# yoshihikosuzuki/ClassPro

Hardware: AMD Instinct MI355X
Metric: Mbases/s classified (k=40, 40x HiFi) at 1/2/4/8 MI355X vs CPU -T16 (higher is better)
Workload: dtype u16/f64

## Files before the change

### classpro_amd/csrc/capi.hip

```cpp
#include <hip/hip_runtime.h>
#include <stdio.h>
#include <stdlib.h>
#include <string.h>
#include <string>
#include <mutex>
#include <vector>
#include <chrono>
#include <thread>
#include <type_traits>
#include <time.h>
#include "cp_host_setup.h"
#include "kernels.hip"

static thread_local std::string g_err;
static int set_err(int code, const std::string &msg) { g_err = msg; return code; }

#define HIPCHK(call)                                                                       \
  do { hipError_t e_ = (call);                                                             \
       if (e_ != hipSuccess)                                                               \
         return set_err(CP_EHIP,std::string(#call)+": "+hipGetErrorString(e_));            \
     } while (0)
static int launch_status() { HIPCHK(hipGetLastError()); return CP_OK; }

extern "C" const char *cp_last_error(void) { return g_err.c_str(); }
// ... 966 lines not shown
  return CP_OK;
}
#endif

#if defined(CP_SEED_DEBUG) || defined(CP_SEED_DEBUG_TAKES)
extern "C" int cp_debug_seed_set(int read)
{ HIPCHK(hipMemcpyToSymbol(HIP_SYMBOL(g_seed_dbg_read),&read,sizeof(int))); return CP_OK; }
extern "C" int cp_debug_seed_get(int *out4, int *recs)
{ HIPCHK(hipDeviceSynchronize());
  HIPCHK(hipMemcpyFromSymbol(out4,HIP_SYMBOL(g_seed_dbg_n),16));
  HIPCHK(hipMemcpyFromSymbol(recs,HIP_SYMBOL(g_seed_dbg),8192*16));
  return CP_OK;
}
#endif
#if defined(CP_SEED_PROF) || defined(CP_PROF_WALK)
static int prof_read(unsigned long long *out, const void *sym, size_t n, bool reset = true)
{ static const unsigned long long z[13] = {0};
  HIPCHK(hipMemcpyFromSymbol(out,sym,n*sizeof(unsigned long long)));
  if (reset) HIPCHK(hipMemcpyToSymbol(sym,z,n*sizeof(unsigned long long)));
  return CP_OK;
}
#endif
#ifdef CP_SEED_PROF
extern "C" int cp_debug_seed_prof(unsigned long long *out8)
{ HIPCHK(hipDeviceSynchronize()); return prof_read(out8,HIP_SYMBOL(g_seed_prof),8); }
#endif
extern "C" int cp_debug_task_counts(cp_workspace *ws, int32_t *out, int64_t nreads)
{ if (!ws || !out || nreads < 0 || nreads > ws->nreads || ws->b.fwc.cap < (size_t)nreads*16)
    return set_err(CP_EINVAL,"cp_debug_task_counts: bad arguments");
  HIPCHK(hipDeviceSynchronize());
  if (nreads > 0) HIPCHK(hipMemcpy(out,ws->b.fwc.p,(size_t)nreads*4*sizeof(int32_t),hipMemcpyDeviceToHost));
  return CP_OK;
}
extern "C" int cp_debug_flag_bytes(cp_workspace *ws, int64_t *out2)
{ if (!ws || !out2) return set_err(CP_EINVAL,"cp_debug_flag_bytes: bad arguments");
  HIPCHK(hipDeviceSynchronize());
  const dbuf *arr[2] = { &ws->b.wall, &ws->b.wall_s };
  for (int a = 0; a < 2; a++)
    { std::vector<uint8_t> h(arr[a]->cap);
      if (arr[a]->cap) HIPCHK(hipMemcpy(h.data(),arr[a]->p,arr[a]->cap,hipMemcpyDeviceToHost));
      int64_t n = 0;
      for (uint8_t v : h) n += v != 0;
      out2[a] = n;
    }
  return CP_OK;
}
#ifdef CP_PROF_WALK
extern "C" int cp_debug_live_prof(unsigned long long *out8)
{ HIPCHK(hipDeviceSynchronize()); return prof_read(out8,HIP_SYMBOL(g_live_prof),8); }
extern "C" int cp_debug_emit_prof(unsigned long long *out8)
{ HIPCHK(hipDeviceSynchronize()); return prof_read(out8,HIP_SYMBOL(g_emit_prof),8); }
extern "C" int cp_debug_fw_prof(unsigned long long *out12)
{ HIPCHK(hipDeviceSynchronize()); return prof_read(out12,HIP_SYMBOL(g_fw_prof),12); }
extern "C" int cp_debug_unrel_prof(unsigned long long *out12)
{ HIPCHK(hipDeviceSynchronize()); return prof_read(out12,HIP_SYMBOL(g_unrel_prof),12); }
extern "C" int cp_debug_rel_prof(unsigned long long *out13)
{ HIPCHK(hipDeviceSynchronize()); return prof_read(out13,HIP_SYMBOL(g_rel_prof),13); }
extern "C" int cp_debug_phase_prof(unsigned long long *out36)
{ HIPCHK(hipDeviceSynchronize());
  CHK(prof_read(out36,HIP_SYMBOL(g_phase_max),12));
  CHK(prof_read(out36+12,HIP_SYMBOL(g_phase_sum),12));
  return prof_read(out36+24,HIP_SYMBOL(g_phase_arg),12,false);
}
#endif

#include "kmer_table.hip"

#include "kmer_counts.hip"

#include "kmer_sort.hip"

#include "kmer_lookup.hip"

#include "kmer_hits.hip"

#include "kmer_runs.hip"

#include "kmer_setops.hip"

#include "kmer_cmphist.hip"

#include "kmer_hetpairs.hip"

#include "kmer_unitigs.hip"

#include "kmer_unitig_graph.hip"

#include "kmer_paths.hip"

#include "kmer_prune.hip"

#include "label_tools.hip"
```

### classpro_amd/csrc/cp_wall.h

```cpp
#pragma once
#include "cp_math.h"
#include "cp_ctx.h"

#ifndef CP_HDM
#ifdef __HIPCC__
#define CP_HDM __host__ __device__ __forceinline__
#else
#define CP_HDM inline
#endif
#endif
#include "cp_bounds.h"

struct cp_perr_dense
  { double *a;
    CP_HDM double get(int pos, int e, int w) const { return a[(size_t)pos*4+e*2+w]; }
    CP_HDM void   set(int pos, int e, int w, double v) { a[(size_t)pos*4+e*2+w] = v; }
    CP_HDM long long cell(int pos, int e, int w) { return (long long)pos*4+e*2+w; }
    CP_HDM double    load(long long c) const { return a[c]; }
    CP_HDM void      store(long long c, double v) { a[c] = v; }
  };

struct cp_perr_hash
  { int32_t *keys;
    double  *vals;
// ... 96 lines not shown
    int                  eidx, oidx;
    int                  overflow;
    int                  use_win = 0, win_base = 0;
    uint64_t             win_lo = 0, win_hi = 0;
    int                  spec_wallnow = 0;
  };

#if defined(CP_PROF_WALK) && defined(__HIP_DEVICE_COMPILE__)
extern __device__ unsigned long long g_live_prof[8];
extern __device__ unsigned long long g_emit_prof[8];
#endif
#if defined(CP_PROF_WALK) && defined(CP_PROF_INNER) && defined(__HIP_DEVICE_COMPILE__)
#define CP_LT(k) do { unsigned long long t_ = wall_clock64(); if (__ffsll((long long)__ballot(1))-1 == (int)(threadIdx.x & 63)) atomicAdd(&g_live_prof[k],t_-lt_); lt_ = wall_clock64(); } while (0)
#define CP_LT0() unsigned long long lt_ = wall_clock64()
#define CP_ET(k) do { unsigned long long t_ = wall_clock64(); if (__ffsll((long long)__ballot(1))-1 == (int)(threadIdx.x & 63)) atomicAdd(&g_emit_prof[k],t_-et_); et_ = wall_clock64(); } while (0)
#define CP_ET0() unsigned long long et_ = wall_clock64()
#else
#define CP_LT(k) ((void)0)
#define CP_LT0() ((void)0)
#define CP_ET(k) ((void)0)
#define CP_ET0() ((void)0)
#endif

#define CP_PERR(R,i,e,w) ((R)->perror.get(i,e,w))
#define CP_NEG_INF (-INFINITY)

template <class RD>
CP_HD void cp_update_perror(RD *R, int i, int e, int w, int cout, int cin, double erate, double lpe, double l1mpe)
{ if (CP_PERR(R,i,e,w) == CP_NEG_INF)
    R->perror.set(i,e,w,cp_p_errorin(R->lf,e,erate,lpe,l1mpe,cout,cin));
}

template <class RD>
CP_HD double cp_logp_diff_pair(const RD *R, int i, int j)
{ const auto &pr = R->prof;
  int n_drop = (int)pr[i-1]-pr[i];
  int n_gain = (int)pr[j]-pr[j-1];
  int cov    = pr[i-1] > pr[j] ? pr[i-1] : pr[j];
  return cp_logp_trans(R->P,i,j,n_drop,n_gain,cov);
}

struct __attribute__((packed, aligned(2))) cp_u16x8 { uint16_t v[8]; };
template <class PROF>
CP_HD cp_u16x8 cp_load_u16x8(const PROF &prof, int lo) { return *reinterpret_cast<const cp_u16x8 *>(CP_SPAN(prof,lo,8)); }

struct __attribute__((packed, aligned(2))) cp_u16x8w { uint32_t w[4]; };
template <class PROF>
CP_HD cp_u16x8w cp_load_u16x8w(const PROF &prof, int lo) { return *reinterpret_cast<const cp_u16x8w *>(CP_SPAN(prof,lo,8)); }
CP_HD int cp_u16x8_get(const cp_u16x8w &x, int q) { return (int)((x.w[q >> 1] >> (16*(q & 1))) & 0xffffu); }

CP_HD bool cp_cthres_ng(int e, int cin, int ct)
{ return (e == CP_SELF) ? (cin >= ct) : (cin < ct); }

struct cp_wall_pre
  { int    cng, wtype, cin, cout, maxt, maxl;
    double maxpe, lpe, l1mpe;
  };

#define CP_CF_LIVE     1
#define CP_CF_WALLNOW  2
#define CP_LC_NONE     0
#define CP_LC_BOUNDARY 1
#define CP_LC_PAIR     2
#define CP_LC_REJECT   3

struct cp_cand_pure
  { double own_pe;
    double lc_v;
    double hc_pe;
    int    lc_j, hc_j;
    int    flags, lc_kind;
  };

template <class RD>
CP_HD void cp_wall_candidate_pre(const RD *R, int i, cp_wall_pre *pre)
{ const cp_dev_params *P = R->P;
  const int cim1 = R->prof[i-1], ci = R->prof[i];
  int cng = cim1-ci;
  if (cng < 0) cng = -cng;
  pre->cng = cng;
  if (cim1 > ci) { pre->wtype = CP_DROP; pre->cin = ci;   pre->cout = cim1; }
  else           { pre->wtype = CP_GAIN; pre->cin = cim1; pre->cout = ci;   }
  int maxt = -1, maxl = -1;
  double maxpe = CP_NEG_INF;
  int l3[3];
  cp_ctx3(R->seq,R->rlen,P->K,pre->wtype,i,l3);
  for (int t = 0; t < 3; t++)
    { int l = l3[t];
      if (l > P->lmax[t]) l = P->lmax[t];
      double pe = P->pe[t][l];
      if (maxpe < pe)
        { maxpe = pe; maxt = t; maxl = l; }
    }
  pre->maxt = maxt; pre->maxl = maxl; pre->maxpe = maxpe;
  pre->lpe = P->lpe[maxt][maxl];
  pre->l1mpe = P->l1mpe[maxt][maxl];
}

CP_HD int cp_wall_candidate_filter(const cp_dev_params *P, int e, const cp_wall_pre &pre)
{ const int CMAX = P->cmax;
  const int cng = pre.cng, cin = pre.cin, cout = pre.cout;
  int ct_init = 0, ct_final = 0;
  if (cout < CMAX)
    { ct_init  = P->cthres[pre.maxt][pre.maxl][cout][CP_INIT][e];
      ct_final = P->cthres[pre.maxt][pre.maxl][cout][CP_FINAL][e];
      if (!(cng > CP_MAX_CNT_CHANGE || cin < (ct_init > 3 ? ct_init : 3)))
        return 0;
    }
  if (e == CP_SELF)
    { if (cout < CMAX && cin >= ct_final)
        return 0;
    }
  else if (cng >= P->cov[CP_HAPLO] || (cout < CMAX && cin < ct_final))
    return CP_CF_WALLNOW;
  return CP_CF_LIVE;
}

struct cp_no_prep { CP_HDM void operator()() const {} };
template <class RD, class PREP>
CP_HD void cp_wall_candidate_live(RD *R, int i, int e, const cp_wall_pre &pre, cp_cand_pure *out, PREP prep)
{ const cp_dev_params *P = R->P;
  const auto &pr = R->prof;
  const int plen = R->plen, K = P->K, CMAX = P->cmax;
  const int w = pre.wtype, cin = pre.cin, cout = pre.cout;
  const int t = pre.maxt, l = pre.maxl;
  out->flags = CP_CF_LIVE; out->lc_kind = CP_LC_NONE; out->lc_j = -1; out->hc_j = -1;
  out->lc_v = out->hc_pe = CP_NEG_INF;
  CP_LT0();
  const int ulen = t+1;
  const bool right = (w == CP_DROP);
  int n, j, cout_j, cin_j;

  const double *nowhere = &P->pe[0][0];
  const double *petab = P->petab;
  const int pe_cmax = P->pe_cmax;
  const double *own_at = cp_p_errorin_at(petab,pe_cmax,e,t,l,cout,cin);
  const double *pei_at = cp_p_errorin_at(petab,pe_cmax,e,CP_HP,1,cout,cin);
  const double own_ld = cp_load_table(own_at ? own_at : nowhere), pei_ld = cp_load_table(pei_at ? pei_at : nowhere);
  const int    thr_i  = P->cthres[CP_HP][1][cout < CMAX ? cout : 0][CP_FINAL][e];
  cp_u16x8w cx;
  const int j0 = right ? (i+K-1) : (i-K+1);
  const int lo8 = right ? j0-2 : j0-(CP_MAX_N_HC+1);
  const bool wide = lo8 >= 0 && lo8+8 <= plen;
  cx.w[0] = cx.w[1] = cx.w[2] = cx.w[3] = 0;
  if (wide) cx = cp_load_u16x8w(pr,lo8);
  prep();
  CP_LT(0);

  const int m = ulen*l;
  n = 0;
  while (true)
    { int idx = right ? i+ulen*(n+1) : i-ulen*(n+1);
      if (right ? (idx >= plen) : (idx <= 0))
        break;
      if (cp_ctx(R->seq,R->rlen,K,w,idx,t) != m+n+1)
        break;
      n++;
    }
  CP_LT(1);
  out->own_pe = own_at ? own_ld : cp_p_errorin_calc(P,e,t,l,cout,cin);
  const int dlc = n-m;
  j = right ? j0+dlc : j0-dlc;
  if (right ? (j <= i) : (j >= i))
    return;

  constexpr int NP = CP_MAX_N_HC+2;
  int pj[NP], pcin[NP], pcout[NP], cw[8];
#ifdef __HIPCC__
// ... 586 lines not shown
```

### classpro_amd/csrc/kernels.hip

```cpp
#include <hip/hip_runtime.h>
#include <stdint.h>
#include <type_traits>
#include "cp_wall.h"
#include "cp_class.h"
#include "cp_seed.h"

#ifdef CP_BOUNDS
__device__ unsigned long long g_bounds[4];
#endif
#define WAVE 64
#define REL_MAXM 1024
#define UNREL_MAXN 1024
#ifndef REL_SMALL_MAXM
#define REL_SMALL_MAXM 112
#endif
#ifndef UNREL_SMALL_MAXN
#define UNREL_SMALL_MAXN 256
#endif
#define GRP_MAX_PLEN 65535

__device__ __forceinline__ void wave_sync() { __syncthreads(); }
__device__ __forceinline__ void wave_sync_lds()
{ __builtin_amdgcn_fence(__ATOMIC_RELEASE,"wavefront"); __builtin_amdgcn_wave_barrier(); __builtin_amdgcn_fence(__ATOMIC_ACQUIRE,"wavefront"); }

__device__ __forceinline__ int lane_id() { return threadIdx.x & (WAVE-1); }
__device__ __forceinline__ int wave_from_below(int v, int first) { return __builtin_amdgcn_update_dpp(first,v,0x138,0xf,0xf,false); }
__device__ __forceinline__ int wave_of_last(int v) { return __builtin_amdgcn_readlane(v,WAVE-1); }

typedef unsigned cp_u4v __attribute__((ext_vector_type(4)));
#ifndef SCAN_PLAIN
__device__ __forceinline__ uint4 scan_load(const uint4 *p)
{ cp_u4v x = __builtin_nontemporal_load(reinterpret_cast<const cp_u4v *>(p)); return make_uint4(x.x,x.y,x.z,x.w); }
#define SCAN_LOAD(p) scan_load(p)
#define SCAN_STORE(p,v) __builtin_nontemporal_store((uint8_t)(v),(p))
#else
#define SCAN_LOAD(p) (*(p))
#define SCAN_STORE(p,v) (*(p) = (uint8_t)(v))
#endif
#ifndef SCAN_UNROLL
#define SCAN_UNROLL 4
#endif
#ifndef SCAN_BLOCKS_PER_CU
#define SCAN_BLOCKS_PER_CU 8
#endif

typedef unsigned short cp_us2 __attribute__((ext_vector_type(2)));
__device__ __forceinline__ unsigned scan_pair_flags(unsigned prevcur, unsigned cur, int rep)
{ const cp_us2 a = __builtin_bit_cast(cp_us2,prevcur), b = __builtin_bit_cast(cp_us2,cur);
  const cp_us2 mn = __builtin_elementwise_min(a,b), mx = __builtin_elementwise_max(a,b);
  const cp_us2 r2 = { (unsigned short)rep, (unsigned short)rep }, two = { 2, 2 }, one = { 1, 1 };
  const cp_us2 s1 = __builtin_elementwise_sub_sat(r2,mn);
  const cp_us2 s2 = __builtin_elementwise_sub_sat((cp_us2)(mx-mn),two);
  const cp_us2 m = __builtin_elementwise_min(__builtin_elementwise_min(s1,s2),one);
  return __builtin_bit_cast(unsigned,m);
}

__global__ void __launch_bounds__(256)
k_scan_candidates(const uint16_t *__restrict__ prof, int64_t total, int rep, uint8_t *__restrict__ bitmap, int64_t nbytes, int has_prev)
{
  const int64_t ngroups = total >> 3;
  const int64_t nthreads = (int64_t)gridDim.x*blockDim.x;
  const int lane = lane_id();
  const uint4 *vp = reinterpret_cast<const uint4 *>(prof);

#ifndef SCAN_INTERLEAVED
  const int64_t wavesz = (int64_t)WAVE*SCAN_UNROLL;
  const int64_t nwaves = nthreads/WAVE;
  const int64_t wid = ((int64_t)blockIdx.x*blockDim.x+threadIdx.x)/WAVE;
  for (int64_t base = wid*wavesz; base < ngroups; base += nwaves*wavesz)
    { uint4 v[SCAN_UNROLL];
      int64_t g[SCAN_UNROLL];
#pragma unroll
      for (int u = 0; u < SCAN_UNROLL; u++)
        { g[u] = base+(int64_t)u*WAVE+lane;
          v[u] = (g[u] < ngroups) ? SCAN_LOAD(&vp[g[u]]) : make_uint4(0,0,0,0);
        }
      unsigned carry = 0;
      if (lane == 0)
        carry = (base > 0 || has_prev) ? prof[base*8-1] : (v[0].x & 0xffff);
#pragma unroll
// ... 17 lines not shown
      int64_t g[SCAN_UNROLL];
#pragma unroll
      for (int u = 0; u < SCAN_UNROLL; u++)
        { g[u] = base+(int64_t)u*blockDim.x+threadIdx.x;
          if (g[u] < ngroups)
            v[u] = SCAN_LOAD(&vp[g[u]]);
          else
            v[u] = make_uint4(0,0,0,0);
        }
#pragma unroll
      for (int u = 0; u < SCAN_UNROLL; u++)
        { const bool live = g[u] < ngroups;
          unsigned last = v[u].w >> 16;
          unsigned prev = __shfl_up(last,1);
          if (lane == 0 && live)
            prev = (g[u] > 0 || has_prev) ? prof[g[u]*8-1] : (v[u].x & 0xffff);
          unsigned c[8] = { v[u].x & 0xffff, v[u].x >> 16, v[u].y & 0xffff, v[u].y >> 16,
                            v[u].z & 0xffff, v[u].z >> 16, v[u].w & 0xffff, v[u].w >> 16 };
          unsigned bits = 0;
#pragma unroll
          for (int k = 0; k < 8; k++)
            { unsigned a = prev, b = c[k];
              unsigned mn = a < b ? a : b, df = a < b ? b-a : a-b;
              bits |= ((mn < (unsigned)rep) && (df >= CP_MIN_CNT_CHANGE)) ? (1u << k) : 0u;
              prev = b;
            }
          if (live)
            SCAN_STORE(&bitmap[g[u]],bits);
        }
    }

#endif

  if (blockIdx.x == 0 && threadIdx.x == 0)
    { int64_t p0 = ngroups << 3;
      if (p0 < total)
        { unsigned bits = 0;
          for (int64_t p = p0; p < total; p++)
            if (p > 0 || has_prev)
              { unsigned a = prof[p-1], b = prof[p];
                unsigned mn = a < b ? a : b, df = a < b ? b-a : a-b;
                if (mn < (unsigned)rep && df >= CP_MIN_CNT_CHANGE) bits |= 1u << (p-p0);
              }
          bitmap[ngroups] = (uint8_t)bits;
          p0 += 8;
        }
      for (int64_t q = p0 >> 3; q < nbytes; q++)
        bitmap[q] = 0;
    }
}

__device__ __forceinline__ uint64_t bitmap_word(const uint64_t *bm, int64_t w, int64_t lo, int64_t hi)
{
  uint64_t x = bm[w];
  int64_t w0 = w << 6;
  if (lo > w0)      x &= ~0ull << (lo-w0);
  if (hi < w0+64)   x &= (hi <= w0) ? 0ull : (~0ull >> (w0+64-hi));
  return x;
}

__global__ void __launch_bounds__(WAVE)
k_count_caps(const uint64_t *__restrict__ bm, const int64_t *__restrict__ prof_off, int nreads,
             int32_t *__restrict__ ncand, int64_t *__restrict__ icap, int64_t *__restrict__ ecap,
             int64_t *__restrict__ hcap)
{ const int r = blockIdx.x;
  if (r >= nreads) return;
  const int lane = lane_id();
  const int64_t lo = prof_off[r]+1, hi = prof_off[r+1];
  int cnt = 0;
  if (hi > lo)
    for (int64_t w = (lo >> 6)+lane; w <= ((hi-1) >> 6); w += WAVE)
      cnt += __popcll(bitmap_word(bm,w,lo,hi));
  for (int o = 32; o > 0; o >>= 1)
    cnt += __shfl_xor(cnt,o);
  if (lane == 0)
    { ncand[r] = cnt;
      icap[r]  = 2*(int64_t)cnt+4;
      ecap[r]  = 16*(int64_t)cnt+64;
      int64_t h = 32;
      while (h < 4*(int64_t)cnt+16) h <<= 1;
      hcap[r] = 2*h;
    }
}

template <class T>
__device__ __forceinline__ T block_scan_excl_256(T x, T *tmp, T *total)
{ const int t = threadIdx.x, lane = t & 63, wv = t >> 6;
  T inc = x;
  for (int o = 1; o < WAVE; o <<= 1)
    { T y = __shfl_up(inc,o); if (lane >= o) inc += y; }
  __syncthreads();
  if (lane == WAVE-1) tmp[wv] = inc;
  __syncthreads();
  T base = 0, all = 0;
#pragma unroll
  for (int w = 0; w < 4; w++) { const T v = tmp[w]; if (w < wv) base += v; all += v; }
  *total = all;
  return base+inc-x;
}

#define SCAN_TILE 1024
#define SCAN_TAG_BITS 24
#define SCAN_TAG_MASK 0xffffffull
struct cp_scan_state { unsigned long long g[3]; unsigned long long pad_; };
__global__ void __launch_bounds__(WAVE)
k_prefix_caps_mb(int64_t *__restrict__ a, int64_t *__restrict__ b, int64_t *__restrict__ c, int n, int64_t *__restrict__ totals,
                 cp_scan_state *__restrict__ state, int epoch, unsigned long long *__restrict__ host_tot)
{ const int t = threadIdx.x, tile = blockIdx.x, i0 = tile*SCAN_TILE+16*t;
  int64_t *arr[3] = { a, b, c };
  int64_t off[3], sum[3], pre[3];
#pragma unroll
// ... 447 lines not shown
          if (mv != ~0ull) break;
        }
      if (nx > 0 && !done && !flush_x(right ? 0x7fffffff : -1)) return;
      if (!done && (right ? plen < jend : jend == 0))
        { const double pe = pe_i * pe_i;
          if (pe >= CP_PE_THRES_FINAL)
            { if (*midx >= R->ecap) { R->overflow = 1; return; }
              ev.wave_grow(*midx);
              if (lane == 0)
                { cp_eintvl x; x.b = right ? i : 0; x.e = right ? plen : i; x.pe = pe;
                  ev.put(*midx,x);
                  F.fo[q] |= CP_W_PAIRED_M;
                }
              (*midx)++;
              if (*midx >= plen) { R->overflow = 8; return; }
            }
        }
      wave_sync();
    }
}

#define CP_PCLS(e,a)   (((uint32_t)(e) << 3) | ((uint32_t)(a) & 7u))
#define CP_PCLS_END(x) ((int)((x) >> 3))
#define CP_PCLS_CLS(x) (((x) & 7u) == 7u ? -1 : (int)((x) & 7u))

struct cp_rrec { int32_t b, e; uint16_t ccb, cce; int32_t idx; double pe; };
static_assert(sizeof(cp_rrec) == 24,"compact reliable-interval record");
struct cp_ivA { int32_t b, e; uint16_t cb, ce, ccb, cce; };
struct cp_ivB { double pe, peo_b, peo_e; };
struct cp_ivC { uint8_t is_rel; int8_t asgn; };
static_assert(sizeof(cp_ivA) == 16 && sizeof(cp_ivB) == 24 && sizeof(cp_ivC) == 2,"interval records as arrays");
struct cp_soa { cp_ivA *a; cp_ivB *b; cp_ivC *c; };
__device__ __forceinline__ void cp_soa_put(const cp_soa &S, int64_t at, const cp_intvl &I)
{ cp_ivA a; a.b = I.b; a.e = I.e; a.cb = I.cb; a.ce = I.ce; a.ccb = I.ccb; a.cce = I.cce;
  cp_ivB b; b.pe = I.pe; b.peo_b = I.peo_b; b.peo_e = I.peo_e;
  cp_ivC c; c.is_rel = I.is_rel; c.asgn = I.asgn;
  S.a[at] = a; S.b[at] = b; S.c[at] = c;
}
__device__ __forceinline__ cp_intvl cp_soa_get(const cp_soa &S, int64_t at)
{ const cp_ivA a = S.a[at]; const cp_ivB b = S.b[at]; const cp_ivC c = S.c[at];
  cp_intvl I;
  memset(&I,0,sizeof(I));
  I.b = a.b; I.e = a.e; I.cb = a.cb; I.ce = a.ce; I.ccb = a.ccb; I.cce = a.cce;
  I.is_rel = c.is_rel; I.asgn = c.asgn; I.pe = b.pe; I.peo_b = b.peo_b; I.peo_e = b.peo_e;
  return I;
}

#ifdef CP_PROF_WALK
__device__ unsigned long long g_phase_max[12], g_phase_sum[12], g_phase_arg[12];
__device__ unsigned long long g_live_prof[8];
__device__ unsigned long long g_unrel_prof[12];
__device__ unsigned long long g_emit_prof[8];
__device__ unsigned long long g_fw_prof[12];
#define EM_LT0() unsigned long long em_t = wall_clock64()
#define EM_LT(k) do { unsigned long long t_ = wall_clock64(); if (lane == 0) atomicAdd(&g_fw_prof[4+(k)],t_-em_t); em_t = wall_clock64(); } while (0)
#define PH_STAMP(k) do { if (lane == 0) { unsigned long long t_ = wall_clock64(); unsigned long long d_ = t_-ph_t; ph_t = t_; \
      atomicAdd(&g_phase_sum[k],d_); unsigned long long o_ = atomicMax(&g_phase_max[k],d_); if (d_ > o_) g_phase_arg[k] = ((unsigned long long)r << 32) | (unsigned)n_c; } } while (0)
#elif defined(CP_STOP_AT)
#define PH_STAMP(k) do { if ((k) == CP_STOP_AT) { PH_STOP_EXTRA; return; } } while (0)
#else
#define PH_STAMP(k) ((void)0)
#endif
#ifndef EM_LT0
#define EM_LT0() ((void)0)
#define EM_LT(k) ((void)0)
#endif
#define PH_STOP_EXTRA

struct task_res { double own_pe, lc_v, hc_pe; int lc_j, hc, pos, kc; };
#define TR_E(hc)     (((hc) >> 3) & 1)
#define TR_WTYPE(hc) (((hc) >> 4) & 1)
static_assert(sizeof(task_res) == 40,"three doubles and four ints, no padding");
static_assert(CP_DROP == 0 && CP_GAIN == 1 && CP_SELF == 0 && CP_OTHERS == 1,"one bit each in task_res::hc");
static_assert(CP_LC_REJECT <= 3,"lc_kind takes two bits of task_res::hc");
struct task_stage { double own_pe, lc_v, hc_pe; int lc_j, hc; };

#define FW_SEQ_WIN    32
#define FW_SEQ_STRIDE 36
struct cp_seq_lwin
  { CP_SEQ_T g; CP_LDS_PTR(const char) w; int lo, len;
    __device__ __forceinline__ char operator[](int p) const
    { const unsigned d = (unsigned)(p-lo); return d < (unsigned)len ? w[d] : g[p]; }
  };
__device__ __forceinline__ int cp_seq_dirword(const cp_seq_lwin &sq, int rlen, int pos, int dir, uint64_t *D)
{ (void)rlen;
  const int d = (dir > 0 ? pos : pos-7)-sq.lo;
  if (d < 0 || d+8 > sq.len) return 0;
  CP_LDS_PTR(const uint32_t) rw = (CP_LDS_PTR(const uint32_t))(sq.w+(d & ~3));
  const uint32_t x0 = rw[0], x1 = rw[1], x2 = rw[2];
  const uint32_t sh = (uint32_t)(d & 3)*8;
  const uint32_t lo = __builtin_amdgcn_alignbit(x1,x0,sh), hi = __builtin_amdgcn_alignbit(x2,x1,sh);
  const uint64_t x = (uint64_t)lo | ((uint64_t)hi << 32);
  *D = dir > 0 ? x : __builtin_bswap64(x);
  return 8;
}
struct __attribute__((packed, aligned(1))) cp_u8x16 { uint32_t v[4]; };
struct __attribute__((packed, aligned(1))) cp_u8x4 { uint32_t v; };
struct cp_seq_rwin
  { CP_SEQ_T g;
    uint64_t wl, wh;
    int lo, len;
    __device__ __forceinline__ char operator[](int p) const
    { const unsigned d = (unsigned)(p-lo);
      if (d < (unsigned)len)
        { const uint64_t x = (d < 8) ? wl : wh;
          return (char)(x >> ((d & 7)*8));
        }
      return g[p];
    }
  };
__device__ __forceinline__ int cp_seq_dirword(const cp_seq_rwin &sq, int rlen, int pos, int dir, uint64_t *D)
{ (void)rlen;
  const int d = (dir > 0 ? pos : pos-7)-sq.lo;
  if (sq.len != 16 || d < 0 || d > 8) return 0;
  const uint64_t x = d == 0 ? sq.wl : d == 8 ? sq.wh : (sq.wl >> (8*d)) | (sq.wh << (64-8*d));
  *D = dir > 0 ? x : __builtin_bswap64(x);
  return 8;
}
struct cp_seq_rsrc { CP_SEQ_T g; };
__device__ __forceinline__ cp_seq_rwin cp_seq_window(const cp_seq_rsrc &src, int pos, int rlen, int dir)
{ cp_seq_rwin sq;
  int lo = dir > 0 ? pos-7 : pos-11;
  if (lo > rlen-16) lo = rlen-16;
  if (lo < 0) lo = 0;
  sq.g = src.g; sq.lo = lo; sq.len = 0; sq.wl = sq.wh = 0;
  if (rlen-lo >= 16)
    { const cp_u8x16 x = *reinterpret_cast<const cp_u8x16 *>(CP_SPAN(src.g,lo,16));
      sq.wl = (uint64_t)x.v[0] | ((uint64_t)x.v[1] << 32);
      sq.wh = (uint64_t)x.v[2] | ((uint64_t)x.v[3] << 32);
      sq.len = 16;
    }
  return sq;
}

#define FR_STRIDE 68
__device__ __forceinline__ void fr_seq_win_load(cp_seq_lwin &sq, char *row, int lo, int rlen)
{ if (lo > rlen-32) lo = rlen-32;
  if (lo < 0) lo = 0;
  const int len = rlen-lo < 32 ? rlen-lo : 32;
  uint32_t *rw = reinterpret_cast<uint32_t *>(row);
  if (len == 32)
    {
#pragma unroll
      for (int k = 0; k < 2; k++)
        { const cp_u8x16 x = *reinterpret_cast<const cp_u8x16 *>(CP_SPAN(sq.g,lo+16*k,16));
          rw[4*k] = x.v[0]; rw[4*k+1] = x.v[1]; rw[4*k+2] = x.v[2]; rw[4*k+3] = x.v[3];
        }
    }
  else
    for (int k = 0; k < len; k++) row[k] = sq.g[lo+k];
  sq.lo = lo; sq.len = len;
}

#ifndef FW_WAVES_PER_EU
#define FW_WAVES_PER_EU 4
#endif
#ifndef FW_LISTS
#define FW_LISTS 255
#endif
#undef PH_STOP_EXTRA
#define PH_STOP_EXTRA do { if (lane == 0) { fwc[4*(int64_t)r] = 0; fwc[4*(int64_t)r+1] = 0; fwc[4*(int64_t)r+2] = 0; fwc[4*(int64_t)r+3] = 0; } } while (0)
__global__ void __launch_bounds__(WAVE) __attribute__((amdgpu_waves_per_eu(FW_WAVES_PER_EU)))
k_wall_tasks(const cp_dev_params *__restrict__ P, const char *__restrict__ seq, const int64_t *__restrict__ seq_off,
             const uint16_t *__restrict__ prof, const int64_t *__restrict__ prof_off, int nreads,
             const uint64_t *__restrict__ bm, uint8_t *__restrict__ wall_all, const int64_t *__restrict__ ioff,
             const int32_t *__restrict__ perm, int32_t *__restrict__ wlist, task_res *__restrict__ tres_all,
             int32_t *__restrict__ fwc)
{ if ((int)blockIdx.x >= nreads) return;
  const int r = perm[blockIdx.x];
  const int lane = lane_id();
  const int64_t po = prof_off[r];
  const int plen = (int)(prof_off[r+1]-po);
  const int rlen = (int)(seq_off[r+1]-seq_off[r]);
  __shared__ __attribute__((aligned(4))) char s_win[WAVE*FW_SEQ_STRIDE];
  static_assert(FW_LISTS <= 255,"the on-chip lists have 256 rows");
  __shared__ int32_t  s_cl[256], s_cc[256];
  __shared__ uint16_t s_ci[256], s_tl[512];
  cp_read_t<cp_perr_hybrid,cp_seq_lwin> R;
  R.P = P; R.prof = CP_PROF_VIEW(prof+po,plen); R.lf = P->logfact; R.plen = plen; R.rlen = rlen;
  R.seq.g = CP_SEQ_VIEW(seq+seq_off[r],rlen); R.seq.w = (CP_LDS_PTR(const char))(s_win+lane*FW_SEQ_STRIDE); R.seq.lo = 0; R.seq.len = 0;
  R.wall = wall_all+po+r; R.wall_s = R.wall;
  R.eintvl = R.ointvl = nullptr; R.ecap = 0; R.eidx = R.oidx = 0; R.overflow = 0;
  cp_read_t<cp_perr_hybrid,cp_seq_rwin> R1;
  R1.P = P; R1.prof = R.prof; R1.lf = P->logfact; R1.plen = plen; R1.rlen = rlen;
  R1.wall = R.wall; R1.wall_s = R.wall; R1.eintvl = R1.ointvl = nullptr; R1.ecap = 0; R1.eidx = R1.oidx = 0; R1.overflow = 0;
  const int icap = (int)(ioff[r+1]-ioff[r]);
  int32_t *wl = wlist+ioff[r]*4;
  task_res *tres = tres_all+ioff[r];
  uint8_t *wall = R.wall;
  int32_t *cinfo = wl, *clist = wl+icap, *ccnt = wl+2*(int64_t)icap, *tlist = wl+3*(int64_t)icap;
  int n_c = 0;
#ifdef CP_PROF_WALK
  unsigned long long ph_t = wall_clock64();
#endif
  if (plen > 1)
    { const int64_t lo = po+1, hi = po+plen;
      const int64_t w_lo = lo >> 6, w_hi = (hi-1) >> 6;
      for (int64_t wb = w_lo; wb <= w_hi; wb += WAVE)
        { const int64_t w = wb+lane;
          const uint64_t bits = (w <= w_hi) ? bitmap_word(bm,w,lo,hi) : 0ull;
          int c = __popcll(bits), off = c;
          for (int o = 1; o < WAVE; o <<= 1)
            { int x = __shfl_up(off,o); if (lane >= o) off += x; }
          const int tot = __shfl(off,WAVE-1);
          off = n_c+off-c;
          for (uint64_t t = bits; t; t &= t-1)
            { const int k = __ffsll((long long)t)-1;
              if (off < icap) clist[off] = (int)((w << 6)+k-po);
              if (off < FW_LISTS) s_cl[off] = (int)((w << 6)+k-po);
              off++;
            }
          n_c += tot;
        }
    }
  if (n_c > icap) n_c = icap;
  const bool lists = n_c <= FW_LISTS;
  if (lists) wave_sync_lds(); else wave_sync();
  PH_STAMP(0);
  int n_t = 0, n_live0 = 0;
  for (int base = 0; base < n_c; base += WAVE)
    { int f0 = 0, f1 = 0;
      if (!lists) { if (base+lane < n_c) s_cl[lane] = clist[base+lane]; wave_sync_lds(); }
      if (base+lane < n_c)
        { const int i = s_cl[lists ? base+lane : lane];
          const bool drop = R.prof[i-1] > R.prof[i];
          cp_seq_rsrc rs; rs.g = R.seq.g;
          R1.seq = cp_seq_window(rs,drop ? i+P->K-2 : i,rlen,drop ? -1 : +1);
          cp_wall_pre pre;
          cp_wall_candidate_pre(&R1,i,&pre);
          f0 = cp_wall_candidate_filter(P,CP_SELF,pre);
          f1 = cp_wall_candidate_filter(P,CP_OTHERS,pre);
          cinfo[base+lane] = pre.maxt*32+pre.maxl+(f0 << 8)+(f1 << 12);
          if (!lists) ccnt[base+lane] = (int)R.prof[i-1] | ((int)R.prof[i] << 16);
          if (lists)
            { s_ci[base+lane] = (uint16_t)(pre.maxt*32+pre.maxl+(f0 << 8)+(f1 << 12));
              s_cc[base+lane] = (int)R.prof[i-1] | ((int)R.prof[i] << 16);
            }
        }
      const int l0 = (f0 & CP_CF_LIVE) ? 1 : 0, l1 = (f1 & CP_CF_LIVE) ? 1 : 0;
      int c = l0+l1, off = c;
      for (int o = 1; o < WAVE; o <<= 1)
        { int x = __shfl_up(off,o); if (lane >= o) off += x; }
      const int tot = __shfl(off,WAVE-1);
      off = n_t+off-c;
      if (l0) { if (lists) s_tl[off] = (uint16_t)((base+lane)*2);   else if (off < icap) tlist[off] = (base+lane)*2;   off++; }
      if (l1) { if (lists) s_tl[off] = (uint16_t)((base+lane)*2+1); else if (off < icap) tlist[off] = (base+lane)*2+1; }
      n_t += tot;
      n_live0 += __popcll(__ballot(l0));
    }
  int ovf = 0;
  if (n_t > icap) { ovf = 1; n_t = 0; n_c = 0; }
  if (lists) wave_sync_lds(); else wave_sync();
  PH_STAMP(7);
  for (int tb = 0; tb < n_t; tb += WAVE)
    { const int nb = (n_t-tb < WAVE) ? n_t-tb : WAVE;
      if (lane < nb)
        { if (!lists)
            { const int code = tlist[tb+lane], k = code >> 1;
              s_tl[lane] = (uint16_t)(lane*2+(code & 1)); s_cl[lane] = clist[k]; s_ci[lane] = (uint16_t)cinfo[k]; s_cc[lane] = ccnt[k];
            }
          const int code = s_tl[lists ? tb+lane : lane], k = code >> 1, e = code & 1;
          const int i = s_cl[k], tl = s_ci[k] & 255, cc = s_cc[k];
          cp_wall_pre pre;
          const int cim1 = cc & 0xffff, ci = (cc >> 16) & 0xffff;
          pre.cng = cim1 > ci ? cim1-ci : ci-cim1;
          if (cim1 > ci) { pre.wtype = CP_DROP; pre.cin = ci;   pre.cout = cim1; }
          else           { pre.wtype = CP_GAIN; pre.cin = cim1; pre.cout = ci;   }
          pre.maxt = tl >> 5; pre.maxl = tl & 31;
          pre.maxpe = P->pe[pre.maxt][pre.maxl];
          pre.lpe   = P->lpe[pre.maxt][pre.maxl];
          pre.l1mpe = P->l1mpe[pre.maxt][pre.maxl];
          cp_cand_pure c;
          cp_wall_candidate_live(&R,i,e,pre,&c,[&]() { fr_seq_win_load(R.seq,s_win+lane*FW_SEQ_STRIDE,cim1 > ci ? i+P->K-16 : i-24,rlen); });
          task_res q;
          q.own_pe = c.own_pe; q.lc_v = c.lc_v; q.hc_pe = c.hc_pe;
          q.lc_j = c.lc_j;
          int code2;
          if (lists) code2 = s_tl[tb+lane]; else code2 = tlist[tb+lane];
          q.hc = c.lc_kind | (c.hc_j >= 0 ? 4 : 0) | ((code2 & 1) << 3) | ((int)pre.wtype << 4)
                 | ((c.hc_j >= 0 ? c.hc_j-i : 0) << 16);
          q.pos = i; q.kc = code2 >> 1;
          tres[tb+lane] = q;
        }
    }
  PH_STAMP(6);
  if (lane == 0) { fwc[4*(int64_t)r] = n_c; fwc[4*(int64_t)r+1] = n_t; fwc[4*(int64_t)r+2] = n_live0; fwc[4*(int64_t)r+3] = ovf; }
}

#undef PH_STOP_EXTRA
#define PH_STOP_EXTRA
#ifndef FW2_WAVES_PER_EU
#define FW2_WAVES_PER_EU 5
#endif
__global__ void __launch_bounds__(WAVE) __attribute__((amdgpu_waves_per_eu(FW2_WAVES_PER_EU)))
k_find_wall(const cp_dev_params *__restrict__ P, const char *__restrict__ seq, const int64_t *__restrict__ seq_off,
            const uint16_t *__restrict__ prof, const int64_t *__restrict__ prof_off, int nreads,
            uint8_t *__restrict__ wall_all, uint8_t *__restrict__ walls_all,
            int32_t *__restrict__ hkeys, double *__restrict__ hvals, const int64_t *__restrict__ hoff,
            cp_eintvl *__restrict__ eintvl_all, cp_eintvl *__restrict__ ointvl_all, const int64_t *__restrict__ eoff,
            cp_intvl *__restrict__ intvl_all, const int64_t *__restrict__ ioff,
            int32_t *__restrict__ nintvl, int32_t *__restrict__ err, const int32_t *__restrict__ perm,
            int32_t *__restrict__ wlist, const task_res *__restrict__ tres_all, const int32_t *__restrict__ fwc,
// ... 2631 lines not shown
```

Measured before the change: 416,200.

## Group candidate bitmap scan per lane and software-pipeline wall prefilter loads

```diff
diff --git a/classpro_amd/csrc/capi.hip b/classpro_amd/csrc/capi.hip
--- a/classpro_amd/csrc/capi.hip
+++ b/classpro_amd/csrc/capi.hip
@@ -1042,6 +1042,8 @@
 { HIPCHK(hipDeviceSynchronize()); return prof_read(out8,HIP_SYMBOL(g_emit_prof),8); }
 extern "C" int cp_debug_fw_prof(unsigned long long *out12)
 { HIPCHK(hipDeviceSynchronize()); return prof_read(out12,HIP_SYMBOL(g_fw_prof),12); }
+extern "C" int cp_debug_p01_prof(unsigned long long *out12)
+{ HIPCHK(hipDeviceSynchronize()); return prof_read(out12,HIP_SYMBOL(g_p01_prof),12); }
 extern "C" int cp_debug_unrel_prof(unsigned long long *out12)
 { HIPCHK(hipDeviceSynchronize()); return prof_read(out12,HIP_SYMBOL(g_unrel_prof),12); }
 extern "C" int cp_debug_rel_prof(unsigned long long *out13)
diff --git a/classpro_amd/csrc/cp_wall.h b/classpro_amd/csrc/cp_wall.h
--- a/classpro_amd/csrc/cp_wall.h
+++ b/classpro_amd/csrc/cp_wall.h
@@ -172,6 +172,67 @@
 CP_HD bool cp_cthres_ng(int e, int cin, int ct)
 { return (e == CP_SELF) ? (cin >= ct) : (cin < ct); }
 
+#define CP_CAND_WPL 8
+CP_HD uint64_t cp_bm_mask(int64_t w, int64_t lo, int64_t hi)
+{ const int64_t w0 = w << 6;
+  uint64_t m = ~0ull;
+  if (lo > w0)    m &= ~0ull << (lo-w0);
+  if (hi < w0+64) m &= (hi <= w0) ? 0ull : (~0ull >> (w0+64-hi));
+  return m;
+}
+CP_HD int cp_cand_wpl(int64_t nwords) { return (int)((nwords+63) >> 6); }
+struct __attribute__((packed, aligned(8))) cp_u64x2 { uint64_t v[2]; };
+struct cp_bm_loads
+  { const uint64_t *bm;
+    CP_HDM uint64_t one(int64_t w) const { return bm[w]; }
+    CP_HDM cp_u64x2 two(int64_t w) const { return *reinterpret_cast<const cp_u64x2 *>(bm+w); }
+  };
+template <class LD>
+CP_HD int64_t cp_cand_lane_fetch(const LD &ld, int64_t lo, int64_t hi, int c, int lane, uint64_t (&x)[CP_CAND_WPL])
+{ const int64_t w_lo = lo >> 6, w_hi = (hi-1) >> 6;
+  const int64_t w0 = w_lo+(int64_t)lane*c;
+  if (c == 1)
+    { x[0] = ld.one(w0 < w_hi ? w0 : w_hi);
+#pragma unroll
+      for (int k = 1; k < CP_CAND_WPL; k++) x[k] = 0;
+    }
+  else
+    { cp_u64x2 v[CP_CAND_WPL/2];
+      int64_t at[CP_CAND_WPL/2];
+#pragma unroll
+      for (int p = 0; p < CP_CAND_WPL/2; p++)
+        { const int64_t a = w0+2*p;
+          at[p] = (2*p < c && a < w_hi) ? a : w_hi-1;
+          v[p] = ld.two(at[p]);
+        }
+#pragma unroll
+      for (int p = 0; p < CP_CAND_WPL/2; p++)
+        { const bool own = at[p] == w0+2*p;
+          x[2*p]   = own ? v[p].v[0] : v[p].v[1];
+          x[2*p+1] = own ? v[p].v[1] : 0ull;
+        }
+    }
+#pragma unroll
+  for (int k = 0; k < CP_CAND_WPL; k++)
+    x[k] = (k < c && w0+k <= w_hi) ? x[k] & cp_bm_mask(w0+k,lo,hi) : 0ull;
+  return w0;
+}
+CP_HD int cp_cand_lane_count(const uint64_t (&x)[CP_CAND_WPL])
+{ int n = 0;
+#pragma unroll
+  for (int k = 0; k < CP_CAND_WPL; k++) n += __builtin_popcountll(x[k]);
+  return n;
+}
+template <class EMIT>
+CP_HD int cp_cand_lane_walk(const uint64_t (&x)[CP_CAND_WPL], int64_t w0, int64_t po, int off, EMIT emit)
+{
+#pragma unroll
+  for (int k = 0; k < CP_CAND_WPL; k++)
+    for (uint64_t t = x[k]; t; t &= t-1)
+      { emit(off,(int)(((w0+k) << 6)+__builtin_ctzll(t)-po)); off++; }
+  return off;
+}
+
 struct cp_wall_pre
   { int    cng, wtype, cin, cout, maxt, maxl;
     double maxpe, lpe, l1mpe;
@@ -217,23 +278,27 @@
   pre->l1mpe = P->l1mpe[maxt][maxl];
 }
 
-CP_HD int cp_wall_candidate_filter(const cp_dev_params *P, int e, const cp_wall_pre &pre)
-{ const int CMAX = P->cmax;
-  const int cng = pre.cng, cin = pre.cin, cout = pre.cout;
-  int ct_init = 0, ct_final = 0;
-  if (cout < CMAX)
-    { ct_init  = P->cthres[pre.maxt][pre.maxl][cout][CP_INIT][e];
-      ct_final = P->cthres[pre.maxt][pre.maxl][cout][CP_FINAL][e];
-      if (!(cng > CP_MAX_CNT_CHANGE || cin < (ct_init > 3 ? ct_init : 3)))
+CP_HD int cp_wall_filter_rule(int CMAX, int cov_haplo, int e, int cng, int cin, int cout, int ct_init, int ct_final)
+{ if (cout < CMAX)
+    { if (!(cng > CP_MAX_CNT_CHANGE || cin < (ct_init > 3 ? ct_init : 3)))
         return 0;
     }
   if (e == CP_SELF)
     { if (cout < CMAX && cin >= ct_final)
         return 0;
     }
-  else if (cng >= P->cov[CP_HAPLO] || (cout < CMAX && cin < ct_final))
+  else if (cng >= cov_haplo || (cout < CMAX && cin < ct_final))
     return CP_CF_WALLNOW;
   return CP_CF_LIVE;
+}
+CP_HD int cp_wall_candidate_filter(const cp_dev_params *P, int e, const cp_wall_pre &pre)
+{ const int CMAX = P->cmax;
+  int ct_init = 0, ct_final = 0;
+  if (pre.cout < CMAX)
+    { ct_init  = P->cthres[pre.maxt][pre.maxl][pre.cout][CP_INIT][e];
+      ct_final = P->cthres[pre.maxt][pre.maxl][pre.cout][CP_FINAL][e];
+    }
+  return cp_wall_filter_rule(CMAX,P->cov[CP_HAPLO],e,pre.cng,pre.cin,pre.cout,ct_init,ct_final);
 }
 
 struct cp_no_prep { CP_HDM void operator()() const {} };
diff --git a/classpro_amd/csrc/kernels.hip b/classpro_amd/csrc/kernels.hip
--- a/classpro_amd/csrc/kernels.hip
+++ b/classpro_amd/csrc/kernels.hip
@@ -26,6 +26,15 @@
 __device__ __forceinline__ int lane_id() { return threadIdx.x & (WAVE-1); }
 __device__ __forceinline__ int wave_from_below(int v, int first) { return __builtin_amdgcn_update_dpp(first,v,0x138,0xf,0xf,false); }
 __device__ __forceinline__ int wave_of_last(int v) { return __builtin_amdgcn_readlane(v,WAVE-1); }
+__device__ __forceinline__ int wave_scan_incl(int x)
+{ x += __builtin_amdgcn_update_dpp(0,x,0x111,0xf,0xf,false);
+  x += __builtin_amdgcn_update_dpp(0,x,0x112,0xf,0xf,false);
+  x += __builtin_amdgcn_update_dpp(0,x,0x114,0xf,0xf,false);
+  x += __builtin_amdgcn_update_dpp(0,x,0x118,0xf,0xf,false);
+  x += __builtin_amdgcn_update_dpp(0,x,0x142,0xa,0xf,false);
+  x += __builtin_amdgcn_update_dpp(0,x,0x143,0xc,0xf,false);
+  return x;
+}
 
 typedef unsigned cp_u4v __attribute__((ext_vector_type(4)));
 #ifndef SCAN_PLAIN
@@ -149,11 +158,7 @@
 
 __device__ __forceinline__ uint64_t bitmap_word(const uint64_t *bm, int64_t w, int64_t lo, int64_t hi)
 {
-  uint64_t x = bm[w];
-  int64_t w0 = w << 6;
-  if (lo > w0)      x &= ~0ull << (lo-w0);
-  if (hi < w0+64)   x &= (hi <= w0) ? 0ull : (~0ull >> (w0+64-hi));
-  return x;
+  return bm[w] & cp_bm_mask(w,lo,hi);
 }
 
 __global__ void __launch_bounds__(WAVE)
@@ -707,6 +712,12 @@
 __device__ unsigned long long g_unrel_prof[12];
 __device__ unsigned long long g_emit_prof[8];
 __device__ unsigned long long g_fw_prof[12];
+__device__ unsigned long long g_p01_prof[12];
+#ifdef CP_PROF_P01
+#define P01_T0() unsigned long long p01_t = wall_clock64()
+#define P01_LT(k) do { __builtin_amdgcn_sched_barrier(0); __builtin_amdgcn_s_waitcnt(0); unsigned long long t_ = wall_clock64(); if (lane == 0) atomicAdd(&g_p01_prof[k],t_-p01_t); p01_t = wall_clock64(); } while (0)
+#define P01_COUNT(k) do { if (lane == 0) atomicAdd(&g_p01_prof[k],1ull); } while (0)
+#endif
 #define EM_LT0() unsigned long long em_t = wall_clock64()
 #define EM_LT(k) do { unsigned long long t_ = wall_clock64(); if (lane == 0) atomicAdd(&g_fw_prof[4+(k)],t_-em_t); em_t = wall_clock64(); } while (0)
 #define PH_STAMP(k) do { if (lane == 0) { unsigned long long t_ = wall_clock64(); unsigned long long d_ = t_-ph_t; ph_t = t_; \
@@ -719,6 +730,11 @@
 #ifndef EM_LT0
 #define EM_LT0() ((void)0)
 #define EM_LT(k) ((void)0)
+#endif
+#ifndef P01_T0
+#define P01_T0() ((void)0)
+#define P01_LT(k) ((void)0)
+#define P01_COUNT(k) ((void)0)
 #endif
 #define PH_STOP_EXTRA
 
@@ -805,6 +821,69 @@
   else
     for (int k = 0; k < len; k++) row[k] = sq.g[lo+k];
   sq.lo = lo; sq.len = len;
+}
+
+#ifndef FW_P0_GROUPED
+#define FW_P0_GROUPED 1
+#endif
+#ifndef FW_1A_GROUPED
+#define FW_1A_GROUPED 1
+#endif
+struct fw_pre_consts { int K, cmax, cov_haplo, lmax[3]; };
+struct fw_pre_loads  { uint32_t cw; cp_u8x16 xd, xg; };
+struct __attribute__((packed, aligned(2))) cp_u16x2w { uint32_t w; };
+__device__ __forceinline__ int fw_win_lo(int pos, int rlen, int dir)
+{ int lo = dir > 0 ? pos-7 : pos-11;
+  if (lo > rlen-16) lo = rlen-16;
+  if (lo < 0) lo = 0;
+  return lo;
+}
+__device__ __forceinline__ void fw_pre_issue(const cp_dev_params *__restrict__ P, const CP_PROF_T &prof, const CP_SEQ_T &seq, int rlen,
+                                             int K, int i, fw_pre_loads &L)
+{ const char *nowhere = reinterpret_cast<const char *>(&P->pe[0][0]);
+  L.cw = reinterpret_cast<const cp_u16x2w *>(CP_SPAN(prof,i-1,2))->w;
+  L.xd = *reinterpret_cast<const cp_u8x16 *>(rlen >= 16 ? CP_SPAN(seq,fw_win_lo(i+K-2,rlen,-1),16) : nowhere);
+  L.xg = *reinterpret_cast<const cp_u8x16 *>(rlen >= 16 ? CP_SPAN(seq,fw_win_lo(i,rlen,+1),16) : nowhere);
+}
+static_assert(offsetof(cp_dev_params,cthres) % 4 == 0 && sizeof(((cp_dev_params *)0)->cthres[0][0][0]) == 4,
+              "the four thresholds of (t, l, cout) are one aligned word");
+struct fw_pre_round2 { int l3[3]; double pe3[3]; uint32_t ct3[3]; };
+__device__ __forceinline__ void fw_pre_ctx(const cp_dev_params *__restrict__ P, const fw_pre_consts &pc, const CP_SEQ_T &seq,
+                                           int rlen, int i, const fw_pre_loads &L, cp_wall_pre *pre, fw_pre_round2 &r2)
+{ const int cim1 = (int)(L.cw & 0xffffu), ci = (int)(L.cw >> 16);
+  const bool drop = cim1 > ci;
+  pre->cng = drop ? cim1-ci : ci-cim1;
+  if (drop) { pre->wtype = CP_DROP; pre->cin = ci;   pre->cout = cim1; }
+  else      { pre->wtype = CP_GAIN; pre->cin = cim1; pre->cout = ci;   }
+  cp_seq_rwin sq;
+  uint32_t x[4];
+#pragma unroll
+  for (int q = 0; q < 4; q++) x[q] = drop ? L.xd.v[q] : L.xg.v[q];
+  sq.g = seq; sq.lo = drop ? fw_win_lo(i+pc.K-2,rlen,-1) : fw_win_lo(i,rlen,+1); sq.len = rlen >= 16 ? 16 : 0;
+  sq.wl = (uint64_t)x[0] | ((uint64_t)x[1] << 32);
+  sq.wh = (uint64_t)x[2] | ((uint64_t)x[3] << 32);
+  if (rlen < 16) sq.wl = sq.wh = 0;
+  cp_ctx3(sq,rlen,pc.K,pre->wtype,i,r2.l3);
+  const int cc = pre->cout < pc.cmax ? pre->cout : 0;
+#pragma unroll
+  for (int t = 0; t < 3; t++)
+    { if (r2.l3[t] > pc.lmax[t]) r2.l3[t] = pc.lmax[t];
+      r2.pe3[t] = cp_load_table(&P->pe[t][r2.l3[t]]);
+      r2.ct3[t] = *reinterpret_cast<const uint32_t *>(&P->cthres[t][r2.l3[t]][cc][0][0]);
+    }
+}
+__device__ __forceinline__ void fw_pre_select(const fw_pre_consts &pc, const fw_pre_round2 &r2, cp_wall_pre *pre, int *f0, int *f1)
+{ int maxt = -1, maxl = -1;
+  double maxpe = CP_NEG_INF;
+  uint32_t ct = 0;
+#pragma unroll
+  for (int t = 0; t < 3; t++)
+    if (maxpe < r2.pe3[t])
+      { maxpe = r2.pe3[t]; maxt = t; maxl = r2.l3[t]; ct = r2.ct3[t]; }
+  pre->maxt = maxt; pre->maxl = maxl; pre->maxpe = maxpe;
+  const int ct_is = ct & 255, ct_io = (ct >> 8) & 255, ct_fs = (ct >> 16) & 255, ct_fo = ct >> 24;
+  *f0 = cp_wall_filter_rule(pc.cmax,pc.cov_haplo,CP_SELF,  pre->cng,pre->cin,pre->cout,ct_is,ct_fs);
+  *f1 = cp_wall_filter_rule(pc.cmax,pc.cov_haplo,CP_OTHERS,pre->cng,pre->cin,pre->cout,ct_io,ct_fo);
 }
 
 #ifndef FW_WAVES_PER_EU
@@ -836,9 +915,6 @@
   R.seq.g = CP_SEQ_VIEW(seq+seq_off[r],rlen); R.seq.w = (CP_LDS_PTR(const char))(s_win+lane*FW_SEQ_STRIDE); R.seq.lo = 0; R.seq.len = 0;
   R.wall = wall_all+po+r; R.wall_s = R.wall;
   R.eintvl = R.ointvl = nullptr; R.ecap = 0; R.eidx = R.oidx = 0; R.overflow = 0;
-  cp_read_t<cp_perr_hybrid,cp_seq_rwin> R1;
-  R1.P = P; R1.prof = R.prof; R1.lf = P->logfact; R1.plen = plen; R1.rlen = rlen;
-  R1.wall = R.wall; R1.wall_s = R.wall; R1.eintvl = R1.ointvl = nullptr; R1.ecap = 0; R1.eidx = R1.oidx = 0; R1.overflow = 0;
   const int icap = (int)(ioff[r+1]-ioff[r]);
   int32_t *wl = wlist+ioff[r]*4;
   task_res *tres = tres_all+ioff[r];
@@ -851,40 +927,123 @@
   if (plen > 1)
     { const int64_t lo = po+1, hi = po+plen;
       const int64_t w_lo = lo >> 6, w_hi = (hi-1) >> 6;
-      for (int64_t wb = w_lo; wb <= w_hi; wb += WAVE)
-        { const int64_t w = wb+lane;
-          const uint64_t bits = (w <= w_hi) ? bitmap_word(bm,w,lo,hi) : 0ull;
-          int c = __popcll(bits), off = c;
-          for (int o = 1; o < WAVE; o <<= 1)
-            { int x = __shfl_up(off,o); if (lane >= o) off += x; }
-          const int tot = __shfl(off,WAVE-1);
-          off = n_c+off-c;
-          for (uint64_t t = bits; t; t &= t-1)
-            { const int k = __ffsll((long long)t)-1;
-              if (off < icap) clist[off] = (int)((w << 6)+k-po);
-              if (off < FW_LISTS) s_cl[off] = (int)((w << 6)+k-po);
-              off++;
-            }
-          n_c += tot;
-        }
+      const int wpl = cp_cand_wpl(w_hi-w_lo+1);
+      P01_T0();
+      if (FW_P0_GROUPED && wpl <= CP_CAND_WPL)
+        { uint64_t x[CP_CAND_WPL];
+          cp_bm_loads ld; ld.bm = bm;
+          const int64_t w0 = cp_cand_lane_fetch(ld,lo,hi,wpl,lane,x);
+          const int c = cp_cand_lane_count(x);
+          P01_LT(0);
+          const int inc = wave_scan_incl(c);
+          n_c = wave_of_last(inc);
+          P01_LT(1);
+          cp_cand_lane_walk(x,w0,po,inc-c,[&](int off, int pos)
+            { if (off < icap) clist[off] = pos;
+              if (off < FW_LISTS) s_cl[off] = pos;
+            });
+          P01_LT(2);
+          P01_COUNT(9);
+        }
+      else
+        for (int64_t wb = w_lo; wb <= w_hi; wb += WAVE)
+          { const int64_t w = wb+lane;
+            const uint64_t bits = (w <= w_hi) ? bitmap_word(bm,w,lo,hi) : 0ull;
+            int c = __popcll(bits), off = c;
+            P01_LT(0);
+            for (int o = 1; o < WAVE; o <<= 1)
+              { int x = __shfl_up(off,o); if (lane >= o) off += x; }
+            const int tot = __shfl(off,WAVE-1);
+            off = n_c+off-c;
+            P01_LT(1);
+            for (uint64_t t = bits; t; t &= t-1)
+              { const int k = __ffsll((long long)t)-1;
+                if (off < icap) clist[off] = (int)((w << 6)+k-po);
+                if (off < FW_LISTS) s_cl[off] = (int)((w << 6)+k-po);
+                off++;
+              }
+            n_c += tot;
+            P01_LT(2);
+          }
     }
   if (n_c > icap) n_c = icap;
+  n_c = __builtin_amdgcn_readfirstlane(n_c);
   const bool lists = n_c <= FW_LISTS;
   if (lists) wave_sync_lds(); else wave_sync();
   PH_STAMP(0);
   int n_t = 0, n_live0 = 0;
+#if FW_1A_GROUPED
+  const fw_pre_consts pc = { P->K, P->cmax, P->cov[CP_HAPLO], { P->lmax[0], P->lmax[1], P->lmax[2] } };
+  auto phase_1a = [&](auto on_chip)
+  { constexpr bool lists = decltype(on_chip)::value;
+    fw_pre_loads cur = {};
+    int i_cur = 1;
+    if (lists && n_c > 0) { i_cur = s_cl[lane < n_c ? lane : n_c-1]; fw_pre_issue(P,R.prof,R.seq.g,rlen,pc.K,i_cur,cur); }
+    for (int base = 0; base < n_c; base += WAVE)
+      { const bool has = base+lane < n_c;
+        P01_T0();
+        if (!lists)
+          { s_cl[lane] = clist[has ? base+lane : n_c-1];
+            wave_sync_lds();
+            i_cur = s_cl[lane];
+            fw_pre_issue(P,R.prof,R.seq.g,rlen,pc.K,i_cur,cur);
+          }
+        const int i = i_cur;
+        P01_LT(3);
+        cp_wall_pre pre;
+        fw_pre_round2 r2;
+        fw_pre_ctx(P,pc,R.seq.g,rlen,i,cur,&pre,r2);
+        const int cc = (int)cur.cw;
+        if (lists)
+          { const int k = base+WAVE+lane;
+            i_cur = s_cl[k < n_c ? k : n_c-1];
+            fw_pre_issue(P,R.prof,R.seq.g,rlen,pc.K,i_cur,cur);
+          }
+        int f0, f1;
+        fw_pre_select(pc,r2,&pre,&f0,&f1);
+        P01_LT(5);
+        if (!has) f0 = f1 = 0;
+        if (has)
+          { cinfo[base+lane] = pre.maxt*32+pre.maxl+(f0 << 8)+(f1 << 12);
+            if (!lists) ccnt[base+lane] = cc;
+            if (lists)
+              { s_ci[base+lane] = (uint16_t)(pre.maxt*32+pre.maxl+(f0 << 8)+(f1 << 12));
+                s_cc[base+lane] = cc;
+              }
+          }
+        const int l0 = (f0 & CP_CF_LIVE) ? 1 : 0, l1 = (f1 & CP_CF_LIVE) ? 1 : 0;
+        const int c = l0+l1, inc = wave_scan_incl(c);
+        int off = n_t+inc-c;
+        if (l0) { if (lists) s_tl[off] = (uint16_t)((base+lane)*2);   else if (off < icap) tlist[off] = (base+lane)*2;   off++; }
+        if (l1) { if (lists) s_tl[off] = (uint16_t)((base+lane)*2+1); else if (off < icap) tlist[off] = (base+lane)*2+1; }
+        n_t += wave_of_last(inc);
+        n_live0 += __popcll(__ballot(l0));
+        P01_LT(7);
+        P01_COUNT(8);
+      }
+  };
+  if (lists) phase_1a(std::true_type()); else phase_1a(std::false_type());
+#else
+  cp_read_t<cp_perr_hybrid,cp_seq_rwin> R1;
+  R1.P = P; R1.prof = R.prof; R1.lf = P->logfact; R1.plen = plen; R1.rlen = rlen;
+  R1.wall = R.wall; R1.wall_s = R.wall; R1.eintvl = R1.ointvl = nullptr; R1.ecap = 0; R1.eidx = R1.oidx = 0; R1.overflow = 0;
   for (int base = 0; base < n_c; base += WAVE)
     { int f0 = 0, f1 = 0;
+      P01_T0();
       if (!lists) { if (base+lane < n_c) s_cl[lane] = clist[base+lane]; wave_sync_lds(); }
       if (base+lane < n_c)
         { const int i = s_cl[lists ? base+lane : lane];
           const bool drop = R.prof[i-1] > R.prof[i];
+          P01_LT(3);
           cp_seq_rsrc rs; rs.g = R.seq.g;
           R1.seq = cp_seq_window(rs,drop ? i+P->K-2 : i,rlen,drop ? -1 : +1);
+          P01_LT(4);
           cp_wall_pre pre;
           cp_wall_candidate_pre(&R1,i,&pre);
+          P01_LT(5);
           f0 = cp_wall_candidate_filter(P,CP_SELF,pre);
           f1 = cp_wall_candidate_filter(P,CP_OTHERS,pre);
+          P01_LT(6);
           cinfo[base+lane] = pre.maxt*32+pre.maxl+(f0 << 8)+(f1 << 12);
           if (!lists) ccnt[base+lane] = (int)R.prof[i-1] | ((int)R.prof[i] << 16);
           if (lists)
@@ -902,7 +1061,10 @@
       if (l1) { if (lists) s_tl[off] = (uint16_t)((base+lane)*2+1); else if (off < icap) tlist[off] = (base+lane)*2+1; }
       n_t += tot;
       n_live0 += __popcll(__ballot(l0));
-    }
+      P01_LT(7);
+      P01_COUNT(8);
+    }
+#endif
   int ovf = 0;
   if (n_t > icap) { ovf = 1; n_t = 0; n_c = 0; }
   if (lists) wave_sync_lds(); else wave_sync();
```

New measurement: 420,400, median of 4. 1.0% higher.
